# sitzikbs/Nesti-Net

Measured on AMD Instinct MI355X. Metric: normals/sec (whole node), synthetic 100k-pt clouds, higher is better.
Workload: dtype f16x8c

## Files before the change

### nesti-net_amd/csrc/nbr_dev.h

```cpp
#pragma once
#include "pca_dev.h"

namespace nesti {
namespace {

constexpr int kNbrTrips = NESTI_KNN_MAX_K / kWave;
static_assert(NESTI_KNN_MAX_K % kWave == 0, "a list is whole trips of the wave");

__device__ __forceinline__ double knn_d2(double dx, double dy, double dz) {
  const double s = dx * dx + dy * dy;
  return s + dz * dz;
}

__device__ __forceinline__ void wave_lds_fence() {
  __builtin_amdgcn_fence(__ATOMIC_RELEASE, "wavefront");
  __builtin_amdgcn_wave_barrier();
  __builtin_amdgcn_fence(__ATOMIC_ACQUIRE, "wavefront");
}

__device__ __forceinline__ int uniform(int v) { return __builtin_amdgcn_readfirstlane(v); }

constexpr int kKnnCap = 1024;
static_assert(NESTI_KNN_MAX_K + kWave <= kKnnCap, "a cut leaves room for the next trip");

__device__ __forceinline__ int knn_cut(double* bd, int* bj, int cnt, int K, int lane) {
  int n2 = kWave;
  while (n2 < cnt) n2 <<= 1;
  for (int i = cnt + lane; i < n2; i += kWave) {
    bd[i] = INFINITY;
    bj[i] = 0x7fffffff;
  }
  wave_lds_fence();
  for (int k = 2; k <= n2; k <<= 1) {
    for (int s = k >> 1; s > 0; s >>= 1) {
      for (int t = lane; t < (n2 >> 1); t += kWave) {
        const int a = ((t & ~(s - 1)) << 1) | (t & (s - 1)), b = a | s;
        const bool up = (a & k) == 0;
        const double da = bd[a], db = bd[b];
        const int ja = bj[a], jb = bj[b];
        const bool a_after_b = da > db || (da == db && ja > jb);
        if (a_after_b == up) {
          bd[a] = db; bd[b] = da;
          bj[a] = jb; bj[b] = ja;
        }
      }
      wave_lds_fence();
    }
  }
  return min(cnt, K);
}

struct NbrParams {
  PatchParams p;
  const int32_t* nbr;
  int K;
  int ks[NESTI_MAX_SCALES];
  float* radius_out;
  int32_t* count_out;
};

template <int S>
__device__ __forceinline__ void nbr_row(const NbrParams& np, int q, int lane, bool lost, int (&j)[kNbrTrips], int (&n)[S]) {
  const int kmax = np.ks[S - 1];
  int bad = lost ? 0 : kmax;
#pragma unroll
  for (int t = 0; t < kNbrTrips; ++t) {
    const int i = lane + t * kWave;
    j[t] = 0;
    if (i < kmax) {
      const int v = np.nbr[(size_t)q * np.K + i];
      if ((unsigned)v >= (unsigned)np.p.N) bad = min(bad, i);
      else j[t] = v;
    }
  }
  bad = wave_min(bad);
#pragma unroll
  for (int s = 0; s < S; ++s) n[s] = min(np.ks[s], bad);
}

__device__ __forceinline__ int nbr_row_upto(const NbrParams& np, int q, int lane, bool lost, int kmax, int (&j)[kNbrTrips]) {
  int bad = lost ? 0 : kmax;
#pragma unroll
  for (int t = 0; t < kNbrTrips; ++t) {
    const int i = lane + t * kWave;
    j[t] = 0;
    if (i < kmax) {
      const int v = np.nbr[(size_t)q * np.K + i];
      if ((unsigned)v >= (unsigned)np.p.N) bad = min(bad, i);
      else j[t] = v;
    }
  }
  return wave_min(bad);
}

struct GroupRow {
  int q, sl;
};
template <int G>
__device__ __forceinline__ GroupRow group_row() {
  static_assert(G == 16 || G == 32 || G == kWave, "a lane group");
  const int lane = threadIdx.x & (kWave - 1);
  const int q = G == kWave ? wave_row() : (int)(blockIdx.x * kRowsPerBlock + (threadIdx.x >> 6)) * (kWave / G) + lane / G;
  return {q, lane & (G - 1)};
}
template <int G>
__device__ __forceinline__ bool group_centre_lost(float x, float y, float z) {
  return G == kWave ? centre_lost(x, y, z) : !(finite_bits(x) && finite_bits(y) && finite_bits(z));
}
template <int G>
__device__ __forceinline__ int group_nbr_row(const NbrParams& np, int q, int sl, bool lost, int (&j)[kNbrTrips]) {
  if constexpr (G == kWave) {
    int ns[1];
    nbr_row<1>(np, q, sl, lost, j, ns);
    return ns[0];
  } else {
    const int k = np.ks[0];
    int bad = lost ? 0 : k;
#pragma unroll
    for (int t = 0; t < kNbrTrips; ++t) j[t] = 0;
    if (sl < k) {
      const int v = np.nbr[(size_t)q * np.K + sl];
      if ((unsigned)v >= (unsigned)np.p.N) bad = sl;
      else j[0] = v;
    }
    return min(min(k, G), group_min<G>(bad));
  }
}

template <class Body>
__device__ __forceinline__ void walk_list(const float* cloud, const int (&j)[kNbrTrips], int n, int lane, double cx, double cy, double cz,
                                          Body&& body) {
#pragma unroll
  for (int t = 0; t < kNbrTrips; ++t) {
    const int i = lane + t * kWave;
    if (i < n) {
      const float* pt = cloud + (size_t)j[t] * 3;
      const double dx = (double)pt[0] - cx, dy = (double)pt[1] - cy, dz = (double)pt[2] - cz;
      body(i, dx, dy, dz, knn_d2(dx, dy, dz));
    }
  }
}


inline int refuse_knn_k(const std::string& w, int K) {
  if (K < 1 || K > NESTI_KNN_MAX_K) NESTI_FAIL(w + ": K must be in 1 .. " + std::to_string(NESTI_KNN_MAX_K));
  return 0;
}

inline int nbr_params_fill(const std::string& w, bool at, NbrParams* np, const float* cloud_dev, int N, const int32_t* query_idx_dev,
                           const float* query_xyz_dev, int M, int query_row0, const int32_t* nbr_dev, int K, const int32_t* ks, int S,
                           float* radius_out_dev, int32_t* count_out_dev) {
  if (!cloud_dev || !nbr_dev || !ks) NESTI_FAIL(w + ": null argument");
  if (N <= 0) NESTI_FAIL(w + ": empty cloud");
  if (refuse_knn_k(w, K)) return 1;
  if (S < 1 || S > NESTI_MAX_SCALES) NESTI_FAIL(w + ": bad n_scales");
  for (int s = 0; s < S; ++s)
    if (ks[s] < 1 || ks[s] > K || (s && ks[s] < ks[s - 1])) NESTI_FAIL(w + ": ks must be ascending and in 1 .. K");
  if (M < 0) NESTI_FAIL(w + ": M must be >= 0");
  if (refuse_query_rows(w, N, !at && !query_idx_dev, M, query_row0)) return 1;
  if (M > 0 && at && !query_xyz_dev) NESTI_FAIL(w + ": null query_xyz_dev");
  memset(np, 0, sizeof(*np));
  np->p.cloud = cloud_dev;
  np->p.query_idx = query_idx_dev;
  np->p.query_xyz = at ? query_xyz_dev : nullptr;
  np->p.M = M; np->p.N = N; np->p.S = S; np->p.row0 = query_row0;
  np->nbr = nbr_dev;
  np->K = K;
  for (int s = 0; s < NESTI_MAX_SCALES; ++s) np->ks[s] = ks[s < S ? s : S - 1];
  np->radius_out = radius_out_dev;
  np->count_out = count_out_dev;
  return 0;
}

}
}
```

### nesti-net_amd/csrc/patches_dev.h

```cpp
#pragma once
#include <string.h>

#include <cmath>
#include <string>

#include "kernels.h"

namespace nesti {
namespace {

constexpr int kMaxDim = 128;
constexpr int kMaxCells = kMaxDim * kMaxDim * kMaxDim;
constexpr int kPatchThreads = 256;
constexpr int kListCap = 1024;

struct GridHeader {
  double minv[3];
  double inv_cell;
  int dims[3];
  int ncells;
};

struct WsLayout {
  size_t header, bbox, count, start, cursor, sorted, total;
};
inline WsLayout patch_ws_layout(int N) {
  WsLayout L;
  size_t o = 0;
  L.header = o; o += 256;
  L.bbox = o; o += 256;
  L.count = o; o += align_up((size_t)(kMaxCells + 1) * 4, 256);
  L.start = o; o += align_up((size_t)(kMaxCells + 1) * 4, 256);
  L.cursor = o; o += align_up((size_t)(kMaxCells + 1) * 4, 256);
  L.sorted = o; o += align_up((size_t)N * 16, 256);
  L.total = o;
  return L;
}

__device__ __forceinline__ int cell_axis(double v, double minv, double inv_cell, int dim) {
  return (int)fmin((double)(dim - 1), fmax(0.0, floor((v - minv) * inv_cell)));
}
__device__ __forceinline__ void cell_coords(const GridHeader& h, float x, float y, float z, int* ix, int* iy, int* iz) {
  *ix = cell_axis((double)x, h.minv[0], h.inv_cell, h.dims[0]);
  *iy = cell_axis((double)y, h.minv[1], h.inv_cell, h.dims[1]);
  *iz = cell_axis((double)z, h.minv[2], h.inv_cell, h.dims[2]);
}
__device__ __forceinline__ int cell_flat(const GridHeader& h, int ix, int iy, int iz) {
  return (iz * h.dims[1] + iy) * h.dims[0] + ix;
}

__device__ __forceinline__ unsigned subsample_hash(unsigned long long seed, unsigned q, unsigned s, unsigned idx) {
  unsigned long long z = seed ^ ((unsigned long long)q << 34) ^ ((unsigned long long)s << 32) ^ (unsigned long long)idx;
  z += 0x9E3779B97F4A7C15ull;
  z = (z ^ (z >> 30)) * 0xBF58476D1CE4E5B9ull;
  z = (z ^ (z >> 27)) * 0x94D049BB133111EBull;
  z = z ^ (z >> 31);
  return (unsigned)(z >> 32);
}

struct PatchParams {
  const float* cloud;
  const float4* sorted;
  const int* start;
  const GridHeader* header;
  const int32_t* query_idx;
  const float* query_xyz;
  int M, N, S, P, row0;
  unsigned long long seed;
  double r2[NESTI_MAX_SCALES];
  float rad_f[NESTI_MAX_SCALES];
  float* points_out;
  int32_t* n_eff_out;
  int32_t* nbr_out;
  int32_t* n_ball_out;
};


struct PatchShared {
  int span_beg[9], span_end[9];
  int s_count[NESTI_MAX_SCALES];
  int s_cnt;
  unsigned long long keys[kListCap];
  int sel[kListCap];
};


__device__ __forceinline__ bool non_finite_bits(float v) {
  unsigned u = __float_as_uint(v);
  asm volatile("" : "+s"(u));
  return (u & 0x7f800000u) == 0x7f800000u;
}
__device__ __forceinline__ bool centre_lost(float x, float y, float z) {
  return non_finite_bits(x) || non_finite_bits(y) || non_finite_bits(z);
}

__device__ __forceinline__ const float* query_centre(const PatchParams& p, int q) {
  if (p.query_xyz) return p.query_xyz + (size_t)q * 3;
  int qi = p.query_idx ? p.query_idx[q] : p.row0 + q;
  qi = min(max(qi, 0), p.N - 1);
  return p.cloud + (size_t)qi * 3;
}

struct Span {
  int b, e;
};
__device__ __forceinline__ Span block_span(const GridHeader& h, const int* start, int N, float x, float y, float z, int t) {
  int ix, iy, iz;
  cell_coords(h, x, y, z, &ix, &iy, &iz);
  const int zz = iz + t / 3 - 1, yy = iy + t % 3 - 1;
  Span s = {0, 0};
  if (zz >= 0 && zz < h.dims[2] && yy >= 0 && yy < h.dims[1]) {
    const int x0 = max(ix - 1, 0), x1 = min(ix + 1, h.dims[0] - 1);
    s.b = max(start[cell_flat(h, x0, yy, zz)], 0);
    s.e = min(start[cell_flat(h, x1, yy, zz) + 1], N);
  }
  return s;
}

struct LdsSpans {
  const int* b;
  const int* e;
  __device__ __forceinline__ Span operator[](int t) const { return {b[t], e[t]}; }
};
struct WaveSpans {
  int b, e;
  __device__ __forceinline__ Span operator[](int t) const { return {__shfl(b, t, 64), __shfl(e, t, 64)}; }
};

__device__ __forceinline__ double ball_d2(double dx, double dy, double dz) {
  return (dx * dx + dy * dy) + dz * dz;
}

template <class Spans, class Body>
__device__ __forceinline__ void walk_block(const float4* sorted, const Spans& spans, int first, int stride, double cx,
                                           double cy, double cz, Body&& body) {
  for (int sp = 0; sp < 9; ++sp) {
    const Span s = spans[sp];
#pragma clang loop unroll(disable) vectorize(disable) interleave(disable)
    for (int i = s.b + first; i < s.e; i += stride) {
      const float4 c = sorted[i];
      body(c, ball_d2((double)c.x - cx, (double)c.y - cy, (double)c.z - cz));
    }
  }
}

__device__ __forceinline__ void patch_query_setup(const PatchParams& p, PatchShared& sh, int q, int t, float (&cf)[3]) {
  const float* centre = query_centre(p, q);
  const GridHeader h = *p.header;
  cf[0] = centre[0]; cf[1] = centre[1]; cf[2] = centre[2];
  const double cx = cf[0], cy = cf[1], cz = cf[2];
  const bool lost = centre_lost(cf[0], cf[1], cf[2]);
  if (t < 9) {
    int b = 0, e = 0;
    if (!lost) {
      int ix, iy, iz;
      cell_coords(h, cf[0], cf[1], cf[2], &ix, &iy, &iz);
      const int zz = iz + t / 3 - 1, yy = iy + t % 3 - 1;
      if (zz >= 0 && zz < h.dims[2] && yy >= 0 && yy < h.dims[1]) {
        const int x0 = max(ix - 1, 0), x1 = min(ix + 1, h.dims[0] - 1);
        b = p.start[cell_flat(h, x0, yy, zz)];
        e = p.start[cell_flat(h, x1, yy, zz) + 1];
      }
    }
    sh.span_beg[t] = b;
    sh.span_end[t] = e;
  }
  if (t < NESTI_MAX_SCALES) sh.s_count[t] = 0;
  __syncthreads();
  int local[NESTI_MAX_SCALES] = {0, 0, 0, 0};
  for (int sp = 0; sp < 9; ++sp) {
    for (int i = sh.span_beg[sp] + t; i < sh.span_end[sp]; i += kPatchThreads) {
      const float4 c = p.sorted[i];
      const double d2 = ball_d2((double)c.x - cx, (double)c.y - cy, (double)c.z - cz);
#pragma unroll
      for (int s = 0; s < NESTI_MAX_SCALES; ++s)
        if (s < p.S && d2 <= p.r2[s]) ++local[s];
    }
  }
#pragma unroll
  for (int s = 0; s < NESTI_MAX_SCALES; ++s)
    if (s < p.S && local[s]) atomicAdd(&sh.s_count[s], local[s]);
  __syncthreads();
}

__device__ __forceinline__ int patch_select_scale(const PatchParams& p, PatchShared& sh, int q, int t, int s, const float (&cf)[3]) {
  const int n_ball = sh.s_count[s];
  const int n_eff = min(n_ball, p.P);
  unsigned lo = 0u, hi = 0xffffffffu, T = 0xffffffffu;
  if (n_ball > p.P) T = (unsigned)fmin(4294967295.0, 4294967296.0 * 1.25 * (double)p.P / (double)n_ball);
  int kept = 0;
  for (int iter = 0; iter < 40; ++iter) {
    __syncthreads();
    if (t == 0) sh.s_cnt = 0;
    __syncthreads();
    walk_block(p.sorted, LdsSpans{sh.span_beg, sh.span_end}, t, kPatchThreads, cf[0], cf[1], cf[2], [&](const float4& c, double d2) {
      if (d2 <= p.r2[s]) {
        const unsigned idx = (unsigned)__float_as_int(c.w);
        const unsigned hsh = subsample_hash(p.seed, (unsigned)(p.row0 + q), (unsigned)s, idx);
        if (hsh <= T) {
          const int pos = atomicAdd(&sh.s_cnt, 1);
          if (pos < kListCap) sh.keys[pos] = ((unsigned long long)hsh << 32) | idx;
        }
      }
    });
    __syncthreads();
    kept = sh.s_cnt;
    if (kept >= n_eff && kept <= kListCap) break;
    if (kept < n_eff) lo = T + 1u; else hi = T - 1u;
    T = lo + (hi - lo) / 2u;
  }
  kept = min(kept, kListCap);
  for (int e = t; e < kept; e += kPatchThreads) {
    const unsigned long long my = sh.keys[e];
    int rank = 0;
    for (int j = 0; j < kept; ++j) rank += (sh.keys[j] < my) ? 1 : 0;
    if (rank < n_eff) sh.sel[rank] = (int)(unsigned)(my & 0xffffffffull);
  }
  __syncthreads();
  return n_eff;
}

__device__ __forceinline__ float patch_coord(const PatchParams& p, int idx, int axis, float c, float rad) {
  return __fdiv_rn(__fsub_rn(p.cloud[(size_t)idx * 3 + axis], c), rad);
}

inline void patch_params_grid(PatchParams* p, int N, const void* grid_ws_dev) {
  const WsLayout L = patch_ws_layout(N);
  const unsigned char* ws = (const unsigned char*)grid_ws_dev;
  p->sorted = (const float4*)(ws + L.sorted);
  p->start = (const int*)(ws + L.start);
  p->header = (const GridHeader*)(ws + L.header);
}

inline void patch_params_fill(PatchParams* p, const nesti_config_t* cfg, const float* cloud_dev, int N,
                              const int32_t* query_idx_dev, int M, const double* r_abs, uint64_t seed, int query_row0,
                              const void* grid_ws_dev) {
  memset(p, 0, sizeof(*p));
  patch_params_grid(p, N, grid_ws_dev);
  p->cloud = cloud_dev;
  p->query_idx = query_idx_dev;
  p->M = M; p->N = N; p->S = cfg->n_scales; p->P = cfg->points_per_scale; p->seed = seed; p->row0 = query_row0;
  for (int s = 0; s < cfg->n_scales; ++s) {
    p->r2[s] = r_abs[s] * r_abs[s];
    p->rad_f[s] = (float)r_abs[s];
  }
}

inline int refuse_grid_cloud(const std::string& w, const nesti_config_t* cfg, const float* cloud_dev, int N, const double* r_abs,
                             const void* grid_ws_dev, size_t grid_ws_bytes, bool radii_used = true) {
  if (!cfg || !cloud_dev || !r_abs || !grid_ws_dev) NESTI_FAIL(w + ": null argument");
  if (N <= 0) NESTI_FAIL(w + ": empty cloud");
  if (cfg->n_scales < 1 || cfg->n_scales > NESTI_MAX_SCALES) NESTI_FAIL(w + ": bad n_scales");
  if (grid_ws_bytes < patch_ws_layout(N).total) NESTI_FAIL(w + ": grid workspace too small");
  for (int s = 0; radii_used && s < cfg->n_scales; ++s)
    if (!(r_abs[s] > 0.0) || !std::isfinite(r_abs[s])) NESTI_FAIL(w + ": radii must be positive and finite");
  return 0;
}
inline int refuse_query_rows(const std::string& w, int N, bool rows_are_centres, int M, int query_row0) {
  if (query_row0 < 0) NESTI_FAIL(w + ": query_row0 must be >= 0");
  if (rows_are_centres && M > 0 && (long long)query_row0 + M > (long long)N)
    NESTI_FAIL(w + ": query rows [query_row0, query_row0 + M) exceed the cloud (N points)");
  return 0;
}

}
}
```

Before: 50900.

## Replace quadratic rank selection with block-wide bitonic sort of subsample keys

```diff
diff --git a/nesti-net_amd/csrc/nbr_dev.h b/nesti-net_amd/csrc/nbr_dev.h
--- a/nesti-net_amd/csrc/nbr_dev.h
+++ b/nesti-net_amd/csrc/nbr_dev.h
@@ -12,11 +12,6 @@
   return s + dz * dz;
 }
 
-__device__ __forceinline__ void wave_lds_fence() {
-  __builtin_amdgcn_fence(__ATOMIC_RELEASE, "wavefront");
-  __builtin_amdgcn_wave_barrier();
-  __builtin_amdgcn_fence(__ATOMIC_ACQUIRE, "wavefront");
-}
 
 __device__ __forceinline__ int uniform(int v) { return __builtin_amdgcn_readfirstlane(v); }
 
diff --git a/nesti-net_amd/csrc/patches_dev.h b/nesti-net_amd/csrc/patches_dev.h
--- a/nesti-net_amd/csrc/patches_dev.h
+++ b/nesti-net_amd/csrc/patches_dev.h
@@ -180,6 +180,45 @@
 #pragma unroll
   for (int s = 0; s < NESTI_MAX_SCALES; ++s)
     if (s < p.S && local[s]) atomicAdd(&sh.s_count[s], local[s]);
+  __syncthreads();
+}
+
+__device__ __forceinline__ void wave_lds_fence() {
+  __builtin_amdgcn_fence(__ATOMIC_RELEASE, "wavefront");
+  __builtin_amdgcn_wave_barrier();
+  __builtin_amdgcn_fence(__ATOMIC_ACQUIRE, "wavefront");
+}
+
+__device__ __forceinline__ void sort_step(unsigned long long* keys, int i, int k, int j) {
+  const int lo = ((i & ~(j - 1)) << 1) | (i & (j - 1)), hi = lo | j;
+  const unsigned long long a = keys[lo], b = keys[hi];
+  const bool up = (lo & k) == 0;
+  if ((a > b) == up) { keys[lo] = b; keys[hi] = a; }
+}
+
+__device__ __forceinline__ void sort_keys(unsigned long long* keys, int n, int t) {
+  if (n < 2) return;
+  int n2 = 2;
+  while (n2 < n) n2 <<= 1;
+  for (int i = n + t; i < n2; i += kPatchThreads) keys[i] = ~0ull;
+  const int lane = t & 63, wave = t >> 6;
+  const int nw = n2 >= 512 ? 4 : (n2 >= 256 ? 2 : 1);
+  const int L = n2 / nw;
+  __syncthreads();
+  for (int k = 2; k <= n2; k <<= 1) {
+    int j = k >> 1;
+    for (; j >= L; j >>= 1) {
+      __syncthreads();
+      for (int i = t; i < (n2 >> 1); i += kPatchThreads) sort_step(keys, i, k, j);
+    }
+    if (k > L) __syncthreads();
+    if (wave < nw) {
+      for (; j > 0; j >>= 1) {
+        for (int i = lane; i < (L >> 1); i += 64) sort_step(keys, wave * (L >> 1) + i, k, j);
+        wave_lds_fence();
+      }
+    }
+  }
   __syncthreads();
 }
 
@@ -210,12 +249,8 @@
     T = lo + (hi - lo) / 2u;
   }
   kept = min(kept, kListCap);
-  for (int e = t; e < kept; e += kPatchThreads) {
-    const unsigned long long my = sh.keys[e];
-    int rank = 0;
-    for (int j = 0; j < kept; ++j) rank += (sh.keys[j] < my) ? 1 : 0;
-    if (rank < n_eff) sh.sel[rank] = (int)(unsigned)(my & 0xffffffffull);
-  }
+  sort_keys(sh.keys, kept, t);
+  for (int r = t; r < n_eff; r += kPatchThreads) sh.sel[r] = (int)(unsigned)(sh.keys[r] & 0xffffffffull);
   __syncthreads();
   return n_eff;
 }
```

Result: no change. 51010, median of 6 (+0.2%).
